# janbruedigam/ConstrainedControl.jl

Hardware: AMD Instinct MI355X
Metric: LQR sim steps/sec (whole node) on N-link cartpole batch (higher is better)
Workload: dtype f64; 1 GPU; lqr_cartpole_n_pendulum N=16 links (17 bodies), hanging-equilibrium LQR, Q=I R=1 horizon 10s, y0~U(-0.5,0.5) phi_i~U(-0.2,0.2); instances_per_gpu=8192, sim_steps=1000, record=True, parallelism=instances sharded x1, lanes_per_instance=32, lds_bytes_per_workgroup=40816, launches_per_rollout=1

## Files before the change

### constrainedcontrol.jl_amd/csrc/cclqr_chain.h

```cpp
#pragma once
#include "cclqr_dev.h"

#if defined(__HIP_DEVICE_COMPILE__)
#define SCHED_FENCE() __builtin_amdgcn_sched_barrier(0)
#else
#define SCHED_FENCE() ((void)0)
#endif
#if defined(__HIP_DEVICE_COMPILE__)
#define LDS_RD(L, i) (*(const volatile __attribute__((address_space(3))) double*)(const __attribute__((address_space(3))) double*)((L) + (i)))
#else
#define LDS_RD(L, i) ((L)[i])
#endif

namespace cclqr {

struct LinkC {
    double m, J[9], p1[3], p2[3], V12[6], qoc[4], axis[3];
    double dtm;
    double sxb, sxa;
    double fric;
    int flags;
    HD bool on() const { return (flags & 1) != 0; }
    HD bool has_a() const { return (flags & 2) != 0; }
    HD bool has_c() const { return (flags & 4) != 0; }
    HD bool rev() const { return (flags & 8) != 0; }
    HD bool valid() const { return (flags & 16) != 0; }
    HD bool live() const { return (flags & 32) != 0; }
    static const int DEAD = 64, BAD = 128;
    static const int FRIC = 256;
    HD bool has_fric() const { return (flags & FRIC) != 0; }
    static const int PRIM = 512;
    HD bool prim() const { return (flags & PRIM) != 0; }
    HD bool dead() const { return (flags & DEAD) != 0; }
    HD bool bad() const { return (flags & BAD) != 0; }
    HD void set_valid(bool v) { flags |= v ? (16 | ((flags & 1) << 5)) : 0; }
};
#if defined(__HIP_DEVICE_COMPILE__)
#define LINK_FLAGS_FRESH(c) asm volatile("" : "+v"((c).flags))
#define LANE_INT_FRESH(x) asm volatile("" : "+v"(x))
#else
#define LINK_FLAGS_FRESH(c) ((void)0)
#define LANE_INT_FRESH(x) ((void)0)
#endif

HD void link_load_consts_rec(LinkC& c, const MechDev* M, const PlantRec* P, int t, int nb, double dt) {
    const bool on = t < nb;
    const int l = on ? t : 0;
    const PlantRec* r = P + l;

    c.m = r->m;
#pragma unroll
    for (int i = 0; i < 9; i++) c.J[i] = r->J[i];
#pragma unroll
    for (int i = 0; i < 3; i++) { c.p1[i] = r->p1[i]; c.p2[i] = r->p2[i]; c.axis[i] = M->axis[l][i]; }
#pragma unroll
    for (int i = 0; i < 4; i++) c.qoc[i] = M->qoc[l][i];
    const int type = M->type[l];
    const int vrow = type == 0 ? 3 : 0;
#pragma unroll
    for (int i = 0; i < 3; i++) { c.V12[i] = M->sel[l][vrow][i]; c.V12[3 + i] = M->sel[l][vrow + 1][i]; }
    const int pa = M->parent[l];
    const bool has_a = on && pa >= 0;
    c.flags = (on ? 1 : 0) | (has_a ? 2 : 0) | ((on && M->childl[l] >= 0) ? 4 : 0) | (type == 0 ? 8 : 0);
    c.dtm = dt / c.m;
    c.sxb = dt * c.dtm;
    c.sxa = has_a ? dt * dt / P[pa >= 0 ? pa : 0].m : 0.0;
    c.fric = 0.0;
}
HD void link_load_consts(LinkC& c, const MechDev* M, int t, int nb, double dt) { link_load_consts_rec(c, M, M->rec, t, nb, dt); }
HD void row_sel(const LinkC& c, int row, double* s) {
    const bool rev = c.rev();
    const int e = rev ? row : row - 2;
    const bool unit = rev ? row < 3 : row >= 2;
    const int v = rev ? row - 3 : row;
#pragma unroll
    for (int i = 0; i < 3; i++) s[i] = unit ? (i == e ? 1.0 : 0.0) : c.V12[3 * (v & 1) + i];
}

template <bool JAC>
HD void joint_eval_sparse(const LinkC& c, const double* xa, const double* qa, const double* xb, const double* qb,
                          const double* Na, const double* Nb, double* g, double (*XT)[3], double (*PB)[3], double (*PA)[3]) {
    double Ra[9], Rb[9], rp[3], w[3], RaTw[3], gT[3];
    rotmat(qa, Ra); rotmat(qb, Rb);
    mv3(Rb, c.p2, rp);
#pragma unroll
    for (int i = 0; i < 3; i++) w[i] = xb[i] + rp[i] - xa[i];
    mtv3(Ra, w, RaTw);
#pragma unroll
    for (int i = 0; i < 3; i++) gT[i] = RaTw[i] - c.p1[i];
    double qac[4] = {qa[0], -qa[1], -qa[2], -qa[3]}, rel[4], e[4];
    qmul(qac, qb, rel);
    qmul(rel, c.qoc, e);
    const bool rot2 = !c.rev();
    if (!JAC) {
#pragma unroll
        for (int row = 0; row < 5; row++) {
            double s[3];
            row_sel(c, row, s);
            const double vT = s[0] * gT[0] + s[1] * gT[1] + s[2] * gT[2], vR = s[0] * e[1] + s[1] * e[2] + s[2] * e[3];
            g[row] = row < 2 ? vT : (row > 2 ? vR : (rot2 ? vR : vT));
        }
        return;
    }
    double RaTRb[9], PTb[9], PRb[9];
    mtm3(Ra, Rb, RaTRb);
    {
        const double* p = c.p2;
#pragma unroll
        for (int i = 0; i < 3; i++) {
            const double a = RaTRb[i * 3], b = RaTRb[i * 3 + 1], cc = RaTRb[i * 3 + 2];
            PTb[i * 3 + 0] = -2.0 * (b * p[2] - cc * p[1]);
            PTb[i * 3 + 1] = -2.0 * (cc * p[0] - a * p[2]);
            PTb[i * 3 + 2] = -2.0 * (a * p[1] - b * p[0]);
        }
    }
    {
        const double s = rel[0], x = rel[1], y = rel[2], z = rel[3];
        const double os = c.qoc[0], ox = c.qoc[1], oy = c.qoc[2], oz = c.qoc[3];
        const double Lr[3][4] = {{x, s, -z, y}, {y, z, s, -x}, {z, -y, x, s}};
        const double Rc[4][3] = {{-ox, -oy, -oz}, {os, oz, -oy}, {-oz, os, ox}, {oy, -ox, os}};
#pragma unroll
        for (int i = 0; i < 3; i++)
#pragma unroll
            for (int j = 0; j < 3; j++) PRb[i * 3 + j] = Lr[i][0] * Rc[0][j] + Lr[i][1] * Rc[1][j] + Lr[i][2] * Rc[2][j] + Lr[i][3] * Rc[3][j];
    }
// ... 167 lines not shown
    inv3(Dr, DINV);
    make_N(w2, sq2, dt, N);
    mm3(N, DINV, NB);
    return acc;
}

#define GKSZ 39
HD int gk_row(int q) { return q < 3 ? 9 * q : 27 + 6 * (q - 3); }

HD void ck_next_pose(const double* z, const double* s, double dt, double* xq) {
    const double* w2 = s + 3;
#pragma unroll
    for (int i = 0; i < 3; i++) xq[i] = z[i] + s[i] * dt;
    const double inv_dt = fast_rcp(dt);
    const double sq2 = sqrt(4.0 * inv_dt * inv_dt - (w2[0] * w2[0] + w2[1] * w2[1] + w2[2] * w2[2]));
    const double wb[4] = {0.5 * dt * sq2, 0.5 * dt * w2[0], 0.5 * dt * w2[1], 0.5 * dt * w2[2]};
    qmul(z + 3, wb, xq + 3);
}

struct SchurCol { double kx[3], kpx[3], kcx[3], kb[3], ka[3], kpb[3], kca[3]; };
HD void schur_col_load(SchurCol& K, int q, int j, int jp, int jc, const Lay& Y, const double* L) {
    const int o = gk_row(q), ob = q < 3 ? 3 : 0;
#pragma unroll
    for (int i = 0; i < 3; i++) {
        if (q < 3) { K.kx[i] = LDS_RD(L, Y.GKA + GKSZ * j + o + i); K.kpx[i] = LDS_RD(L, Y.GKA + GKSZ * jp + o + i); K.kcx[i] = LDS_RD(L, Y.GKA + GKSZ * jc + o + i); }
        else { K.kx[i] = 0.0; K.kpx[i] = 0.0; K.kcx[i] = 0.0; }
        K.kb[i] = LDS_RD(L, Y.GKA + GKSZ * j + o + ob + i); K.ka[i] = LDS_RD(L, Y.GKA + GKSZ * j + o + ob + 3 + i);
        K.kpb[i] = LDS_RD(L, Y.GKA + GKSZ * jp + o + ob + i); K.kca[i] = LDS_RD(L, Y.GKA + GKSZ * jc + o + ob + 3 + i);
    }
}
template <bool PF = false>
HD void ck_schur_rows(const LinkC& c, int j, bool store, const Lay& Y, double* L, const double (*wXT)[3], const double (*wPB)[3],
                      const double (*wPA)[3], const double* g, const double* d, const double* pd) {
    const double sx = c.sxb + c.sxa;
    const int jp = c.has_a() ? j - 1 : j, jc = c.has_c() ? j + 1 : j;
    SchurCol KA, KB;
    if (PF) schur_col_load(KA, 0, j, jp, jc, Y, L);
#pragma unroll
    for (int q = 0; q < 5; q++) {
        SchurCol& K = PF ? ((q & 1) ? KB : KA) : KA;
        if (!PF) schur_col_load(K, q, j, jp, jc, Y, L);
        else if (q < 4) { schur_col_load((q & 1) ? KA : KB, q + 1, j, jp, jc, Y, L); SCHED_FENCE(); }
        const double *kx = K.kx, *kpx = K.kpx, *kcx = K.kcx, *kb = K.kb, *ka = K.ka, *kpb = K.kpb, *kca = K.kca;
        double ojj[5], ojp[5], ojc[5];
#pragma unroll
        for (int r = 0; r < 5; r++) {
            const double bb = wPB[r][0] * kb[0] + wPB[r][1] * kb[1] + wPB[r][2] * kb[2];
            const double aa = wPA[r][0] * ka[0] + wPA[r][1] * ka[1] + wPA[r][2] * ka[2];
            const double ajp = wPA[r][0] * kpb[0] + wPA[r][1] * kpb[1] + wPA[r][2] * kpb[2];
            const double bjc = wPB[r][0] * kca[0] + wPB[r][1] * kca[1] + wPB[r][2] * kca[2];
            if (r < 3 && q < 3) {
                const double xx = wXT[r][0] * kx[0] + wXT[r][1] * kx[1] + wXT[r][2] * kx[2];
                const double xjp = wXT[r][0] * kpx[0] + wXT[r][1] * kpx[1] + wXT[r][2] * kpx[2];
                const double xjc = wXT[r][0] * kcx[0] + wXT[r][1] * kcx[1] + wXT[r][2] * kcx[2];
                ojj[r] = sx * xx + bb + aa; ojp[r] = ajp - c.sxa * xjp; ojc[r] = bjc - c.sxb * xjc;
            } else { ojj[r] = bb + aa; ojp[r] = ajp; ojc[r] = bjc; }
        }
        if (store) {
#pragma unroll
            for (int r = 0; r < 5; r++) L[Y.SJJ + 25 * j + 5 * q + r] = ojj[r];
            if (c.has_a()) {
#pragma unroll
                for (int r = 0; r < 5; r++) L[Y.SJP + 25 * j + 5 * q + r] = ojp[r];
            }
            if (c.has_c()) {
#pragma unroll
                for (int r = 0; r < 5; r++) L[Y.SPJ + 25 * jc + 5 * q + r] = ojc[r];
            }
        }
        SCHED_FENCE();
    }
    if (store) {
#pragma unroll
        for (int r = 0; r < 5; r++) {
            const double bd = wPB[r][0] * d[3] + wPB[r][1] * d[4] + wPB[r][2] * d[5];
            const double ad = wPA[r][0] * pd[3] + wPA[r][1] * pd[4] + wPA[r][2] * pd[5];
            double rr = g[r] - bd - ad;
            if (r < 3) {
                const double xd = wXT[r][0] * d[0] + wXT[r][1] * d[1] + wXT[r][2] * d[2];
                const double xa = wXT[r][0] * pd[0] + wXT[r][1] * pd[1] + wXT[r][2] * pd[2];
                rr = g[r] - (c.sxb * xd + bd) - (ad - c.sxa * xa);
            }
            L[Y.R + 5 * j + r] = rr;
        }
    }
}

template <int KL> struct SubRows { static const int NR = KL == 3 ? 2 : 3; };
struct SubSel {
    double sa[3], sb[3], s2[3];
    int w;
    int ia, ib, ic;
};
HD void row_sel_rt(const LinkC& c, int row, double* s) {
    const bool rev = c.rev();
    const bool unit = rev ? row < 3 : row >= 2;
    const int e = rev ? row : row - 2, v = rev ? row - 3 : row;
#pragma unroll
    for (int i = 0; i < 3; i++) s[i] = unit ? (i == e ? 1.0 : 0.0) : c.V12[3 * (v & 1) + i];
}
template <int KL>
HD void sub_setup(const LinkC& c, int w, SubSel& Q) {
    Q.w = w;
    const bool mid = KL == 3 && w == 2;
    row_sel_rt(c, 2, Q.s2);
    row_sel_rt(c, mid ? 2 : (w & 1), Q.sa);
    row_sel_rt(c, mid ? 2 : 3 + (w & 1), Q.sb);
    Q.ia = mid ? 2 : w;
    Q.ib = mid ? -1 : 3 + w;
    Q.ic = (KL == 2 && w == 0) ? 2 : -1;
}
template <int KL>
HD void joint_eval_rows(const LinkC& c, const SubSel& Q, const double* xa, const double* qa, const double* xb, const double* qb, const double* Na, const double* Nb,
                        double* g, double (*XT)[3], double (*PB)[3], double (*PA)[3]) {
    constexpr int NR = SubRows<KL>::NR;
    double Ra[9], Rb[9], rp[3], wv[3], RaTw[3], gT[3];
    rotmat(qa, Ra); rotmat(qb, Rb);
    mv3(Rb, c.p2, rp);
#pragma unroll
    for (int i = 0; i < 3; i++) wv[i] = xb[i] + rp[i] - xa[i];
    mtv3(Ra, wv, RaTw);
#pragma unroll
    for (int i = 0; i < 3; i++) gT[i] = RaTw[i] - c.p1[i];
    double qac[4] = {qa[0], -qa[1], -qa[2], -qa[3]}, rel[4], e[4];
    qmul(qac, qb, rel);
    qmul(rel, c.qoc, e);
    double RaTRb[9], PTb[9], PRb[9];
    mtm3(Ra, Rb, RaTRb);
    {
        const double* p = c.p2;
#pragma unroll
        for (int i = 0; i < 3; i++) {
            const double a = RaTRb[i * 3], b = RaTRb[i * 3 + 1], cc = RaTRb[i * 3 + 2];
            PTb[i * 3 + 0] = -2.0 * (b * p[2] - cc * p[1]);
            PTb[i * 3 + 1] = -2.0 * (cc * p[0] - a * p[2]);
            PTb[i * 3 + 2] = -2.0 * (a * p[1] - b * p[0]);
        }
    }
    {
        const double s = rel[0], x = rel[1], y = rel[2], z = rel[3];
        const double os = c.qoc[0], ox = c.qoc[1], oy = c.qoc[2], oz = c.qoc[3];
        const double Lr[3][4] = {{x, s, -z, y}, {y, z, s, -x}, {z, -y, x, s}};
        const double Rc[4][3] = {{-ox, -oy, -oz}, {os, oz, -oy}, {-oz, os, ox}, {oy, -ox, os}};
#pragma unroll
        for (int i = 0; i < 3; i++)
#pragma unroll
            for (int j = 0; j < 3; j++) PRb[i * 3 + j] = Lr[i][0] * Rc[0][j] + Lr[i][1] * Rc[1][j] + Lr[i][2] * Rc[2][j] + Lr[i][3] * Rc[3][j];
    }
    const double PTa[9] = {0, -2 * RaTw[2], 2 * RaTw[1], 2 * RaTw[2], 0, -2 * RaTw[0], -2 * RaTw[1], 2 * RaTw[0], 0};
    const double PRa[9] = {-e[0], -e[3], e[2], e[3], -e[0], -e[1], -e[2], e[1], -e[0]};
    const bool rot2 = !c.rev();
    double pb3[NR][3], pa3[NR][3];
    {
        const double a0 = Q.sa[0], a1 = Q.sa[1], a2 = Q.sa[2], b0 = Q.sb[0], b1 = Q.sb[1], b2 = Q.sb[2];
        const double vT = a0 * gT[0] + a1 * gT[1] + a2 * gT[2], vR = b0 * e[1] + b1 * e[2] + b2 * e[3];
        int wq = Q.w;
        LANE_INT_FRESH(wq);
        const bool merge = KL == 3 && wq == 2;
        const bool rot = merge && rot2;
        g[0] = rot ? vR : vT;
        g[1] = merge ? 0.0 : vR;
#pragma unroll
        for (int k = 0; k < 3; k++) {
            const double xt = a0 * Ra[k * 3] + a1 * Ra[k * 3 + 1] + a2 * Ra[k * 3 + 2];
            const double ptb = a0 * PTb[k] + a1 * PTb[3 + k] + a2 * PTb[6 + k], pta = a0 * PTa[k] + a1 * PTa[3 + k] + a2 * PTa[6 + k];
            const double prb = b0 * PRb[k] + b1 * PRb[3 + k] + b2 * PRb[6 + k], pra = b0 * PRa[k] + b1 * PRa[3 + k] + b2 * PRa[6 + k];
// ... 438 lines not shown
```

### constrainedcontrol.jl_amd/csrc/rollout_chain.hip

```cpp
#include "cclqr_chain.h"
#include "cclqr_internal.h"
#include "cclqr_newton.h"
#include "cclqr_rollout_step.h"

namespace cclqr {

__device__ __forceinline__ double wave_from_prev(double v) {
    int lo = __double2loint(v), hi = __double2hiint(v);
    lo = __builtin_amdgcn_update_dpp(0, lo, 0x138, 0xf, 0xf, true);
    hi = __builtin_amdgcn_update_dpp(0, hi, 0x138, 0xf, 0xf, true);
    return __hiloint2double(hi, lo);
}
__device__ __forceinline__ double wave_from_next(double v) {
    int lo = __double2loint(v), hi = __double2hiint(v);
    lo = __builtin_amdgcn_update_dpp(0, lo, 0x130, 0xf, 0xf, true);
    hi = __builtin_amdgcn_update_dpp(0, hi, 0x130, 0xf, 0xf, true);
    return __hiloint2double(hi, lo);
}
template <int N>
__device__ __forceinline__ void from_prev(const double* in, double* out) {
#pragma unroll
    for (int i = 0; i < N; i++) out[i] = wave_from_prev(in[i]);
}
template <int N>
__device__ __forceinline__ void from_next(const double* in, double* out) {
#pragma unroll
    for (int i = 0; i < N; i++) out[i] = wave_from_next(in[i]);
}

__device__ __forceinline__ void ck_tri_mid_regs(int t, bool done, const TriPlanB& B, const TriCur& K, const Lay& Y, const double* L, const double* tg, double* dl, TriBack0& Q) {
    const TriPlan& P = B.P;
    ck_tri_back0_load(Q, t, done, B, K, Y, L);
    double m[5];
    const bool ran = K.n == P.steps;
#pragma unroll
    for (int r = 0; r < 5; r++) m[r] = ran ? tg[r] : 0.0;
    if (P.steps == 0) {
        asm volatile("");
        const bool f0 = (t & 8) == 0;
#pragma unroll
        for (int r = 0; r < 5; r++) m[r] = f0 ? Q.z[r] : 0.0;
    }
#pragma unroll
    for (int r = 0; r < 5; r++) m[r] = m[r] + dpp_row_ror<8>(m[r]);
    double A[25];
#pragma unroll
    for (int i = 0; i < 5; i++) {
        A[i * 5 + 0] = dpp_f64<0x150>(m[i]); A[i * 5 + 1] = dpp_f64<0x151>(m[i]); A[i * 5 + 2] = dpp_f64<0x152>(m[i]);
        A[i * 5 + 3] = dpp_f64<0x153>(m[i]); A[i * 5 + 4] = dpp_f64<0x154>(m[i]);
        dl[i] = dpp_f64<0x155>(m[i]);
    }
    lu5_factor(A);
    lu5_solve(A, dl);
}

template <int G, bool JAC, int KL = 1>
__device__ __forceinline__ double chain_eval(LinkC& c, LinkS& S, int t, const Lay& Y, double* L, double alpha, bool active, bool rows, double dt, const SubSel& Q PROF_ARG) {
    double part = 0.0;
    double NB[9], g[5], xq[7];
    const bool store_dinv = JAC && __any(rows);
    LINK_FLAGS_FRESH(c);
#pragma unroll
    for (int k = 0; k < 7; k++) xq[k] = S.z[k];
    if (active) {
        double cf[6], sv[6], cTR[6], DINV[9];
#pragma unroll
        for (int k = 0; k < 6; k++) { cf[k] = L[Y.C + 6 * t + k] - alpha * S.cd[k]; sv[k] = S.s[k] - alpha * S.ds[k]; cTR[k] = L[Y.D + 6 * t + k]; }
        part = ck_body_eval<JAC>(c, S.z, sv, cf, cTR, cTR + 3, dt, xq, S.d, DINV, NB);
        if (KL > 1 && !c.prim()) part = 0.0;
        if (store_dinv && (KL == 1 || c.prim())) {
#pragma unroll
            for (int k = 0; k < 9; k++) L[Y.DINV + 9 * t + k] = DINV[k];
        }
    }
    STAMP(PF_EVAL_BODY);
    double pxq[7], pNB[9];
    from_prev<7>(xq, pxq);
    if (JAC) from_prev<9>(NB, pNB);
    if (!c.has_a()) {
#pragma unroll
        for (int i = 0; i < 7; i++) pxq[i] = (i == 3) ? 1.0 : 0.0;
    }
    if (JAC && KL > 1) {
        constexpr int NR = SubRows<KL>::NR;
        double gs[NR], sXT[NR][3], sPB[NR][3], sPA[NR][3];
        if (active) {
            joint_eval_rows<KL>(c, Q, pxq, pxq + 3, xq, xq + 3, pNB, NB, gs, sXT, sPB, sPA);
#pragma unroll
            for (int i = 0; i < NR; i++) part += gs[i] * gs[i];
        }
        STAMP(PF_EVAL_JOINT);
        LINK_FLAGS_FRESH(c);
        if (__any(rows)) {
            double pd[6];
            from_prev<6>(S.d, pd);
            ck_schur_rows_sub<KL, (KL == 3)>(c, Q, t, active, Y, L, gs, sXT, sPB, sPA, S.d, pd);
        } else {
            PCOUNT(PF_ROWS_SKIPPED);
        }
        STAMP(PF_SCHUR_S);
    } else {
        double wXT[3][3], wPB[5][3], wPA[5][3];
        if (active) {
            joint_eval_sparse<JAC>(c, pxq, pxq + 3, xq, xq + 3, pNB, NB, g, wXT, wPB, wPA);
            if (KL == 1) {
#pragma unroll
                for (int i = 0; i < 5; i++) part += g[i] * g[i];
            } else {
                double pj = 0.0;
#pragma unroll
                for (int i = 0; i < 5; i++) pj += g[i] * g[i];
                part += c.prim() ? pj : 0.0;
            }
        }
        STAMP(PF_EVAL_JOINT);
        LINK_FLAGS_FRESH(c);
        if (JAC) {
            if (__any(rows)) {
                double pd[6];
                from_prev<6>(S.d, pd);
                ck_schur_rows(c, t, active, Y, L, wXT, wPB, wPA, g, S.d, pd);
            } else {
                PCOUNT(PF_ROWS_SKIPPED);
            }
            STAMP(PF_SCHUR_S);
        }
    }
    const double nrm = sqrt(group_sum<G>(part));
    STAMP(PF_EVAL_MAP);
    PCOUNT(PF_EVALS);
    return nrm;
}

template <int G, int KL = 1>
__device__ __forceinline__ void chain_eval2(LinkC& c, const TrialIn& T, const double* Lc, int t, const Lay& Y, double a1, double a2, bool active, double dt,
                                            double& n1, double& n2) {
    double part1 = 0.0, part2 = 0.0, xq1[7], xq2[7];
    LINK_FLAGS_FRESH(c);
#pragma unroll
    for (int k = 0; k < 7; k++) { xq1[k] = T.z[k]; xq2[k] = T.z[k]; }
    if (active) {
        double cf1[6], cf2[6], sv1[6], sv2[6], cTR[6], d1[6], d2[6];
#pragma unroll
        for (int k = 0; k < 6; k++) {
            const double cc = Lc[Y.C + 6 * t + k];
            cTR[k] = Lc[Y.D + 6 * t + k];
            cf1[k] = cc - a1 * T.cd[k]; cf2[k] = cc - a2 * T.cd[k];
            sv1[k] = T.s[k] - a1 * T.ds[k]; sv2[k] = T.s[k] - a2 * T.ds[k];
        }
        part1 = ck_body_eval<false>(c, T.z, sv1, cf1, cTR, cTR + 3, dt, xq1, d1, nullptr, nullptr);
        part2 = ck_body_eval<false>(c, T.z, sv2, cf2, cTR, cTR + 3, dt, xq2, d2, nullptr, nullptr);
    }
    double p1[7], p2[7];
    from_prev<7>(xq1, p1);
    from_prev<7>(xq2, p2);
    if (!c.has_a()) {
#pragma unroll
        for (int i = 0; i < 7; i++) { p1[i] = (i == 3) ? 1.0 : 0.0; p2[i] = p1[i]; }
    }
    if (active) {
        double g1[5], g2[5];
        joint_eval_sparse<false>(c, p1, p1 + 3, xq1, xq1 + 3, nullptr, nullptr, g1, (double(*)[3]) nullptr, (double(*)[3]) nullptr, (double(*)[3]) nullptr);
        joint_eval_sparse<false>(c, p2, p2 + 3, xq2, xq2 + 3, nullptr, nullptr, g2, (double(*)[3]) nullptr, (double(*)[3]) nullptr, (double(*)[3]) nullptr);
#pragma unroll
        for (int i = 0; i < 5; i++) { part1 += g1[i] * g1[i]; part2 += g2[i] * g2[i]; }
    }
    if (KL > 1 && !c.prim()) { part1 = 0.0; part2 = 0.0; }
    n1 = sqrt(group_sum<G>(part1));
    n2 = sqrt(group_sum<G>(part2));
}

template <int G, int KL = 1>
__device__ __forceinline__ double chain_eval1(LinkC& c, const TrialIn& T, const double* Lc, int t, const Lay& Y, double a1, bool active, double dt) {
    double part1 = 0.0, xq1[7];
    LINK_FLAGS_FRESH(c);
#pragma unroll
    for (int k = 0; k < 7; k++) xq1[k] = T.z[k];
    if (active) {
        double cf1[6], sv1[6], cTR[6], d1[6];
#pragma unroll
        for (int k = 0; k < 6; k++) {
            cTR[k] = Lc[Y.D + 6 * t + k];
            cf1[k] = Lc[Y.C + 6 * t + k] - a1 * T.cd[k];
            sv1[k] = T.s[k] - a1 * T.ds[k];
        }
        part1 = ck_body_eval<false>(c, T.z, sv1, cf1, cTR, cTR + 3, dt, xq1, d1, nullptr, nullptr);
    }
    double p1[7];
    from_prev<7>(xq1, p1);
    if (!c.has_a()) {
#pragma unroll
        for (int i = 0; i < 7; i++) p1[i] = (i == 3) ? 1.0 : 0.0;
    }
    if (active) {
        double g1[5];
        joint_eval_sparse<false>(c, p1, p1 + 3, xq1, xq1 + 3, nullptr, nullptr, g1, (double(*)[3]) nullptr, (double(*)[3]) nullptr, (double(*)[3]) nullptr);
#pragma unroll
        for (int i = 0; i < 5; i++) part1 += g1[i] * g1[i];
    }
    if (KL > 1 && !c.prim()) part1 = 0.0;
    return sqrt(group_sum<G>(part1));
}
__device__ __forceinline__ double lane_fetch(double v, int addr) {
    return __hiloint2double(__builtin_amdgcn_ds_bpermute(addr, __double2hiint(v)), __builtin_amdgcn_ds_bpermute(addr, __double2loint(v)));
}

__device__ __attribute__((noinline)) double philox_normal_dev(unsigned key0, unsigned long long instance, int k) { return philox_normal(key0, instance, k); }
__global__ __launch_bounds__(256) void philox_fill_kernel(double* out, unsigned key0, long long inst0, long long n_inst, int k0, int steps) {
    const long long i = (long long)blockIdx.x * 256 + threadIdx.x;
    if (i >= n_inst * steps) return;
    const long long n = i / steps;
    const int kk = (int)(i - n * steps);
    out[i] = philox_normal_dev(key0, (unsigned long long)(inst0 + n), k0 + kk);
}
hipError_t launch_philox_fill(double* out, unsigned key0, long long inst0, long long n_inst, int k0, int steps, hipStream_t stream) {
    const long long total = n_inst * steps;
    if (total <= 0) return hipSuccess;
    return launch_lds<false>(philox_fill_kernel, dim3((unsigned)((total + 255) / 256)), dim3(256), 0, stream, out, key0, inst0, n_inst, k0, steps);
}

template <int G, int NBP, int EXTRA, bool RELAX = false, int KL = 1, int NL = G>
__global__ __launch_bounds__(WAVE_BLOCK) void rollout_chain_kernel(RolloutArgs a) {
    extern __shared__ double lds[];
    static_assert(WAVE_BLOCK == 64, "WAVE_HANDOVER orders the phases of ONE wavefront: the workgroup is exactly 64 threads");
    static_assert(KL >= 1 && KL <= 3 && KL * NL <= G && (KL > 1 || NL == G) && (KL == 1 || NL <= NBP), "lane group too small for KL lanes per link");
    const int lane = threadIdx.x, t = lane % G, grp = lane / G;
    const int w = KL > 1 ? t / NL : 0;
    const int tl = KL > 1 ? t - NL * w : t;
    const int tc = KL > 1 ? (w < KL ? tl : -2) : t;
    const int64_t inst = (int64_t)blockIdx.x * a.ipw + grp;
    const MechDev* M = a.M;
    const CtrlDev* CT = a.C;
    const int nb = M->nb;
    const double dt = M->dt;
    const Lay Y = make_chain_layout(NBP);
    double* L = lds + grp * Y.total;
    const int nz = 13 * nb;

    LinkC c;
    const PlantRec* plant = M->rec;
    const bool have = grp < a.ipw && inst < a.n_inst;
    if (a.plants) plant = a.plants + ((unsigned)a.plant_off + (have ? (unsigned)inst : 0u)) * (unsigned)nb;
    link_load_consts_rec(c, M, plant, (KL > 1 && w >= KL) ? CCLQR_MAXL : tl, nb, dt);
    if (KL == 1 || w == 0) c.flags |= LinkC::PRIM;
    SubSel Q;
    if (KL > 1) sub_setup<KL>(c, w < KL ? w : 0, Q);
    if (EXTRA && CT->has_fric && c.on()) { c.fric = CT->fric[tl]; if (c.fric != 0.0) c.flags |= LinkC::FRIC; }
    c.set_valid(have);
    const long long ginst = a.inst0 + inst;
    const int ut = c.on() ? M->perm[tl] : 0;
    int plan;
    {
        const int nch = M->nchains;
        const int cs = M->chain_start[lane], cn = M->chain_len[lane];
        plan = chain_plan_pack(nch, lane < nch ? cs : 0, lane < nch ? cn : 0) | (ut << 24);
    }

    LinkS S;
    double pid_int = 0.0, pid_last = 0.0;
#pragma unroll
    for (int i = 0; i < 7; i++) S.z[i] = c.live() ? a.z0[inst * nz + ut * 13 + i] : ((i == 3) ? 1.0 : 0.0);
#pragma unroll
    for (int i = 0; i < 6; i++) S.s[i] = c.live() ? a.z0[inst * nz + ut * 13 + 7 + i] : 0.0;
    if (EXTRA == 2 && a.pid_state && a.k0 > 1 && c.live()) { pid_int = a.pid_state[(inst * nb + tl) * 2]; pid_last = a.pid_state[(inst * nb + tl) * 2 + 1]; }
#pragma unroll
    for (int i = 0; i < 6; i++) { S.cd[i] = 0.0; S.d[i] = 0.0; S.ds[i] = 0.0; }
    if (c.on() && (KL == 1 || c.prim())) {
        const bool warm = c.live() && a.lam && a.k0 > 1;
#pragma unroll
        for (int i = 0; i < 5; i++) L[Y.LAM + 5 * tl + i] = warm ? a.lam[inst * 5 * nb + 5 * tl + i] : 0.0;
    }
    WAVE_HANDOVER();

#ifdef CCLQR_PROFILE
    Prof prof;
    prof.start();
#endif
    int worst = 0;
    if (a.carry && a.status && c.valid()) {
        const NewtonStatus st = status_decode(a.status[inst]);
        worst = st.worst;
        if (st.bad) c.flags |= LinkC::BAD;
        if (st.dead) c.flags |= LinkC::DEAD;
    }
    typedef const __attribute__((address_space(4))) RolloutArgs* KernArgs;
    KernArgs ap = (KernArgs)__builtin_amdgcn_kernarg_segment_ptr();
    const int k0 = a.k0;
    int nsteps = a.steps;
    for (int kk = 0; kk < nsteps; kk++) {
        const int k = k0 + kk;
        asm volatile("" : "+s"(ap));
        LINK_FLAGS_FRESH(c);
        CtrlHotK C = ctrl_hot_of(CT);
        asm volatile("" : "+s"(C));
        const long long gi = c.valid() ? ginst : a.inst0;
        const int ne = 12 * nb;
        const int mu = C->mu;
        const CtrlRows rows = ctrl_step_rows(C, k, gi, nz, ne);
        const bool gate = rows.gate;
        const GlobalD Kp = global_table(C->K) + rows.K + t;
        const GlobalD Fp = C->Fd ? global_table(C->Fd) + rows.Fd : (GlobalD)0;
        double grav = M->g;
        unsigned long long zd_base = C->zd;
        asm volatile("" : "+s"(zd_base));
        double* const traj_out = ap->traj;
        if (traj_out) {
            if (c.live() && (KL == 1 || c.prim())) {
                LANE_INT_FRESH(plan);
                const int ub = plan >> 24;
#pragma unroll
                for (int i = 0; i < 7; i++) L[Y.Z + 13 * ub + i] = S.z[i];
#pragma unroll
                for (int i = 0; i < 6; i++) L[Y.Z + 13 * ub + 7 + i] = S.s[i];
            }
        }
        STAMP(PF_IO);
        double uj = 0.0;
        double zf[13], za[13];
#pragma unroll
        for (int i = 0; i < 7; i++) zf[i] = S.z[i];
#pragma unroll
        for (int i = 0; i < 6; i++) zf[7 + i] = S.s[i];
        from_prev<7>(zf, za);
        if (EXTRA) from_prev<6>(zf + 7, za + 7);
        if (!c.has_a()) {
#pragma unroll
            for (int i = 0; i < 13; i++) za[i] = (i == 3) ? 1.0 : 0.0;
// ... 9 lines not shown
#pragma unroll
                    for (int i = 0; i < 12; i++) L[Y.DZ + 12 * tl + i] = dz[i];
                }
                if (EXTRA && (C->flags & CtrlHot::FRIC) && c.has_fric()) uj = ck_friction(c, zf, za);
            }
        }
        WAVE_HANDOVER();
        if (gate) {
            constexpr int NE = GainRows<G, NBP>::NE;
            double unoise = 0.0;
            if (EXTRA == 3) {
                if (C->flags & CtrlHot::NOISE) unoise = C->noise_scale * philox_normal_dev(C->noise_key0, (unsigned long long)gi, k);
            } else if (EXTRA) {
                const double* noise = ap->noise;
                if ((C->flags & CtrlHot::NOISE) && c.valid() && noise) unoise = C->noise_scale * noise[(size_t)inst * ap->noise_stride + (k - 1)];
            }
            double dzv[NE];
            int tf = t;
            asm volatile("" : "+v"(tf));
#pragma unroll
            for (int q = 0; q < NE; q++) { const int e = tf + q * G; dzv[q] = (c.valid() && e < ne) ? L[Y.DZ + e] : 0.0; }
            feedback_inputs<G, NBP, EXTRA>(C, Kp, Fp, mu, ne, dzv, unoise, tc, uj);
        }
        STAMP(PF_CONTROL);
        asm volatile("" : "+v"(grav));
        if (traj_out) {
            if (c.valid()) {
                int kr = kk, nzr = nz;
                asm volatile("" : "+s"(kr), "+s"(nzr));
                double* dst = traj_out + ((size_t)inst * ap->steps + kr) * nzr;
                int e0 = t;
                asm volatile("" : "+v"(e0));
                for (int e = e0; e < nz; e += G) dst[e] = L[Y.Z + e];
            }
        }
        STAMP(PF_IO);
        if (EXTRA == 2 && (C->flags & CtrlHot::PID)) {
            if (c.live() && CT->pid_on[tl]) uj += ck_pid(c, zf, za, CT->pid_P[tl], CT->pid_I[tl], CT->pid_D[tl], CT->pid_goal[tl], dt, k == 1, pid_int, pid_last);
        }
        STAMP(PF_CONTROL);
        LINK_FLAGS_FRESH(c);
        {
            double F[3], tau[3], W6[6], cW6[6];
            ck_joint_wrench(c, uj, zf + 3, za + 3, F, tau, W6, W6 + 3);
            from_next<6>(W6, cW6);
            if (c.has_c()) {
#pragma unroll
                for (int i = 0; i < 3; i++) { F[i] += cW6[i]; tau[i] += cW6[3 + i]; }
            }
            double cTR[6];
            ck_step_invariants(c, zf, F, tau, dt, grav, cTR, cTR + 3);
            double gk[5], kXT[3][3], kPB[5][3], kPA[5][3], lam[5];
            joint_eval_sparse<true>(c, za, za + 3, zf, zf + 3, nullptr, nullptr, gk, kXT, kPB, kPA);
#pragma unroll
            for (int i = 0; i < 5; i++) lam[i] = L[Y.LAM + 5 * tl + i];
            if (c.live() && (KL == 1 || c.prim())) {
                gk_store(tl, Y, L, kXT, kPB, kPA);
#pragma unroll
                for (int i = 0; i < 6; i++) L[Y.D + 6 * tl + i] = cTR[i];
            }
            double own[6], par[6], cpar[6];
            jac_t_apply(c, kXT, kPB, kPA, lam, own, par);
            from_next<6>(par, cpar);
#pragma unroll
            for (int i = 0; i < 6; i++) S.cd[i] = 0.0;
            if (c.live() && (KL == 1 || c.prim())) {
#pragma unroll
                for (int i = 0; i < 6; i++) L[Y.C + 6 * tl + i] = own[i] + (c.has_c() ? cpar[i] : 0.0);
            }
        }
        WAVE_HANDOVER();

        STAMP(PF_FORCES);
        PCOUNT(PF_STEPS);
        const bool go = c.valid() && !c.dead();
        bool done = !go, failed = false;
        int its = 0;
        double normf0 = 0.0;
        LANE_INT_FRESH(plan);
        const int nchains = chain_plan_count(__builtin_amdgcn_readfirstlane(plan));
        bool need_jac = !done;
        for (int iter = 1; iter <= NEWTON_MAXIT; iter++) {
            if (__any(need_jac)) {
                const double nf = chain_eval<G, true, KL>(c, S, tl, Y, L, 0.0, c.live() && need_jac, need_jac, dt, Q PROF_PASS);
                if (iter == 1) normf0 = nf;
            }
            WAVE_HANDOVER();
            if (!__any(!done)) break;
            PCOUNT(PF_NEWTON_ITERS);
            const bool active = c.live() && !done;
            for (int ci = 0; ci < nchains; ci++) {
                const int pw = __builtin_amdgcn_readlane(plan, ci);
                const int cs = chain_plan_start(pw), cn = chain_plan_len(pw);
                constexpr int CRW = 4;
                constexpr bool CR = G == 32 && NBP <= 17;
                const bool cr = CR && cn >= CR_MIN_LINKS;
                if (CR && cr) {
                    CrLane<CRW> CK;
                    double tc[CrLane<CRW>::NS][5];
                    cr_setup<CRW>(CK, t, cs, cn, 1, Y, done);
                    CR_FLAGS_FRESH(CK);
                    cr_phase_a<CRW>(CK, L, tc);
                    CR_FLAGS_FRESH(CK);
                    cr_store_a<CRW>(CK, L, tc);
                    WAVE_HANDOVER();
                    CR_FLAGS_FRESH(CK);
                    cr_phase_b<CRW>(CK, L, tc);
                    CR_FLAGS_FRESH(CK);
                    cr_store_b<CRW>(CK, L, tc);
                    WAVE_HANDOVER();
                }
                STAMP(PF_SCHUR_W);
                const TriPlanB PB = cr ? tri_plan_balanced(cs, (cn + 1) / 2, 2) : tri_plan_balanced(cs, cn, 1, G >= 16 ? 2 : 1);
                const TriPlan& P = PB.P;
                TriCur K = tri_cursor(t, PB, Y);
                if (done) K.n = 0;
                if constexpr (G >= 16) {
                    double tg[5] = {0.0, 0.0, 0.0, 0.0, 0.0}, dlm[5];
                    for (int i = 0; i < P.steps; i++) {
                        double zy[5];
                        int otg = 0, oout = 0;
                        int left = P.steps - 1 - i;
                        LANE_INT_FRESH(left);
                        if (tri_step(K, i, L, tg, zy, &otg, &oout)) tri_step_store_fold(L, otg, oout, tg, zy, left == 0);
                        WAVE_HANDOVER();
                    }
                    STAMP(PF_TRI_FWD);
                    TriBack0 B0;
                    ck_tri_mid_regs(t, done, PB, K, Y, L, tg, dlm, B0);
                    ck_tri_back0_store(B0, t, Y, L, dlm);
                    WAVE_HANDOVER();
                    for (int j = 1; j < P.steps; j++) {
                        if (!done) ck_tri_back(t, j, PB, Y, L);
                        WAVE_HANDOVER();
                    }
                    if (!done && t == 0) {
#pragma unroll
                        for (int i = 0; i < 5; i++) L[Y.DL + 5 * P.mid + i] = dlm[i];
                    }
                    WAVE_HANDOVER();
                } else {
                    for (int i = 0; i < P.steps; i++) {
                        double tg[5], zy[5];
                        int otg = 0, oout = 0;
                        if (tri_step(K, i, L, tg, zy, &otg, &oout)) tri_step_store(L, otg, oout, tg, zy);
                        WAVE_HANDOVER();
                    }
                    STAMP(PF_TRI_FWD);
                    if (!done) ck_tri_mid<false>(t, PB, Y, L);
                    WAVE_HANDOVER();
                    for (int j = 0; j < P.steps; j++) {
                        if (!done) ck_tri_back(t, j, PB, Y, L);
                        WAVE_HANDOVER();
                    }
                }
                if (CR && cr) {
                    cr_back<CRW>(t, cs, cn, 1, Y, L, done);
                    WAVE_HANDOVER();
                }
                STAMP(PF_TRI_BWD);
            }
            double nd;
            LINK_FLAGS_FRESH(c);
            {
                double own[6], par[6], cpar[6], dl[5], pdn = 0.0;
#pragma unroll
                for (int r = 0; r < 5; r++) dl[r] = L[Y.DL + 5 * tl + r];
                gk_t_apply<true>(c, tl, Y, L, dl, own, par);
                from_next<6>(par, cpar);
                if (active) {
                    double DINV[9];
#pragma unroll
                    for (int i = 0; i < 9; i++) DINV[i] = L[Y.DINV + 9 * tl + i];
#pragma unroll
                    for (int i = 0; i < 6; i++) S.cd[i] = own[i] + (c.has_c() ? cpar[i] : 0.0);
                    ck_body_solve(c, S.d, S.cd, DINV, S.ds);
#pragma unroll
                    for (int i = 0; i < 6; i++) pdn += S.ds[i] * S.ds[i];
#pragma unroll
                    for (int i = 0; i < 5; i++) pdn += dl[i] * dl[i];
                    if (KL > 1 && !c.prim()) pdn = 0.0;
                }
                nd = sqrt(group_sum<G>(pdn));
            }
            WAVE_HANDOVER();
            STAMP(PF_BODY_SOLVE);
            double alpha = 1.0, normf1 = 0.0;
            const bool want_rows = !done && !(normf0 < NEWTON_EPS && nd < NEWTON_EPS);
            bool ls_done = done, jac_ok = __any(want_rows);
            {
                const double nf = chain_eval<G, true, KL>(c, S, tl, Y, L, 1.0, active, want_rows, dt, Q PROF_PASS);
                if (!ls_done) {
                    normf1 = nf;
                    if (!(normf1 > normf0)) ls_done = true;
                }
            }
            if (G == 32) {
                for (int lv = 1; lv <= LINE_MAXIT;) {
                    if (!__any(!ls_done)) break;
                    const bool mine = !ls_done;
                    const bool other = __shfl_xor(mine ? 1 : 0, 32, 64) != 0;
                    const bool solo = ap->plants != nullptr;
                    const bool helping = !mine && other && !solo;
                    TrialIn T;
#pragma unroll
                    for (int i = 0; i < 7; i++) T.z[i] = S.z[i];
#pragma unroll
                    for (int i = 0; i < 6; i++) { T.s[i] = S.s[i]; T.ds[i] = S.ds[i]; T.cd[i] = S.cd[i]; }
                    if (mine != other) {
#pragma unroll
                        for (int i = 0; i < 7; i++) { const double o = other_half(S.z[i]); T.z[i] = helping ? o : T.z[i]; }
#pragma unroll
                        for (int i = 0; i < 6; i++) {
                            const double o1 = other_half(S.s[i]), o2 = other_half(S.ds[i]), o3 = other_half(S.cd[i]);
                            T.s[i] = helping ? o1 : T.s[i]; T.ds[i] = helping ? o2 : T.ds[i]; T.cd[i] = helping ? o3 : T.cd[i];
                        }
                    }
                    const double* Lc = helping ? lds + (1 - grp) * Y.total : L;
                    const int l0 = helping ? lv + 2 : lv;
                    double n1, n2;
                    chain_eval2<G, KL>(c, T, Lc, tl, Y, ldexp(1.0, -l0), ldexp(1.0, -(l0 + 1)), c.on() && (mine || helping) && l0 <= LINE_MAXIT, dt, n1, n2);
                    PCOUNT(PF_EVALS);
                    const double h1 = other_half(n1), h2 = other_half(n2);
                    if (mine) {
                        const double cand[4] = {n1, n2, h1, h2};
#pragma unroll
                        for (int i = 0; i < 4; i++) {
                            const int l = lv + i;
                            if (!ls_done && l <= LINE_MAXIT && (i < 2 || !(other || solo))) {
                                normf1 = cand[i]; alpha = ldexp(1.0, -l); jac_ok = false;
                                if (!(cand[i] > normf0) || l == LINE_MAXIT) ls_done = true;
                            }
                        }
                    }
                    lv += (solo || (mine && other)) ? 2 : 4;
                }
            } else {
                constexpr int NG = 64 / G;
                for (int lv = 1; lv <= LINE_MAXIT;) {
                    if (!__any(!ls_done)) break;
                    const bool mine = !ls_done;
                    const unsigned long long heads = __ballot(mine && t == 0);
                    const bool solo = ap->plants != nullptr;
                    const int count = solo ? NG : __builtin_popcountll(heads);
                    const int per = NG / count;
                    const int kq = grp % count, off = grp / count;
                    unsigned long long hm = heads;
                    for (int i = 0; i < kq; i++) hm &= hm - 1;
                    const int src = solo ? grp : __builtin_ctzll(hm) / G;
                    int myrank = 0;
                    for (int g2 = 0; g2 < NG; g2++) myrank += (g2 < grp && ((heads >> (g2 * G)) & 1ull)) ? 1 : 0;
                    const int l0 = lv + off;
                    const bool work = off < per && l0 <= LINE_MAXIT;
                    const int fa = (src * G + t) * 4;
                    TrialIn T;
#pragma unroll
                    for (int i = 0; i < 7; i++) T.z[i] = S.z[i];
#pragma unroll
                    for (int i = 0; i < 6; i++) { T.s[i] = S.s[i]; T.ds[i] = S.ds[i]; T.cd[i] = S.cd[i]; }
                    if (count < NG) {
#pragma unroll
                        for (int i = 0; i < 7; i++) T.z[i] = lane_fetch(S.z[i], fa);
#pragma unroll
                        for (int i = 0; i < 6; i++) { T.s[i] = lane_fetch(S.s[i], fa); T.ds[i] = lane_fetch(S.ds[i], fa); T.cd[i] = lane_fetch(S.cd[i], fa); }
                    }
                    const double nf = chain_eval1<G, KL>(c, T, lds + src * Y.total, tl, Y, ldexp(1.0, -l0), c.on() && work, dt);
                    PCOUNT(PF_EVALS);
                    if (count == NG) {
                        if (mine) {
                            normf1 = nf; alpha = ldexp(1.0, -lv); jac_ok = false;
                            if (!(nf > normf0) || lv == LINE_MAXIT) ls_done = true;
                        }
                    } else {
#pragma unroll
// ... 137 lines not shown
```

Baseline: 28.95 million instance-steps/s.

## Split Schur row assembly across idle lanes in 32-lane chain groups

For 17-body chains on 32-lane groups, idle upper lanes become helpers that take half of each link's Schur-complement block work. Joint Jacobian weights are swapped across 16-lane rows with permlane16_swap, and a new split routine writes the diagonal and off-diagonal blocks from separate lanes. The aim is to shorten the per-lane critical path of the row assembly. In exchange it adds cross-lane swaps, a root special case and more complex indexing, which risks register pressure and correctness issues.

```diff
diff --git a/constrainedcontrol.jl_amd/csrc/cclqr_chain.h b/constrainedcontrol.jl_amd/csrc/cclqr_chain.h
--- a/constrainedcontrol.jl_amd/csrc/cclqr_chain.h
+++ b/constrainedcontrol.jl_amd/csrc/cclqr_chain.h
@@ -31,6 +31,9 @@
     HD bool has_fric() const { return (flags & FRIC) != 0; }
     static const int PRIM = 512;
     HD bool prim() const { return (flags & PRIM) != 0; }
+    static const int HELP = 1024, HELPC = 2048;
+    HD bool help() const { return (flags & HELP) != 0; }
+    HD bool help_c() const { return (flags & HELPC) != 0; }
     HD bool dead() const { return (flags & DEAD) != 0; }
     HD bool bad() const { return (flags & BAD) != 0; }
     HD void set_valid(bool v) { flags |= v ? (16 | ((flags & 1) << 5)) : 0; }
@@ -38,9 +41,11 @@
 #if defined(__HIP_DEVICE_COMPILE__)
 #define LINK_FLAGS_FRESH(c) asm volatile("" : "+v"((c).flags))
 #define LANE_INT_FRESH(x) asm volatile("" : "+v"(x))
+#define LANE_F64_FRESH(x) asm volatile("" : "+v"(x))
 #else
 #define LINK_FLAGS_FRESH(c) ((void)0)
 #define LANE_INT_FRESH(x) ((void)0)
+#define LANE_F64_FRESH(x) ((void)0)
 #endif
 
 HD void link_load_consts_rec(LinkC& c, const MechDev* M, const PlantRec* P, int t, int nb, double dt) {
@@ -374,6 +379,81 @@
                 rr = g[r] - (c.sxb * xd + bd) - (ad - c.sxa * xa);
             }
             L[Y.R + 5 * j + r] = rr;
+        }
+    }
+}
+
+HD void schur_split_helper(LinkC& c, bool has_child, double sxb_link) {
+    c.flags |= LinkC::HELP | (has_child ? LinkC::HELPC : 0);
+    c.sxb = -sxb_link; c.sxa = -0.0;
+}
+template <bool R0>
+HD void ck_schur_rows_split(const LinkC& c, int t, bool store, bool gstore, const Lay& Y, double* L, const double (*wXT)[3], const double (*wPB)[3],
+                            double (*wPA)[3], const double* g, const double* d, const double* pd) {
+    const bool help = c.help(), root = R0 && t == 0, plain = !help && !root;
+    const int jc = t - (help ? 16 : 0) + ((c.flags >> (help ? 11 : 2)) & 1);
+    const int j1 = help ? jc : t, j3 = plain ? t - ((c.flags >> 1) & 1) : jc;
+    const int x1 = Y.GKA + GKSZ * j1, p1 = x1 + (help ? 3 : 0);
+    const int x3 = Y.GKA + GKSZ * j3, p3 = x3 + (root ? 3 : 0);
+    const int o1 = (help ? Y.SPJ : Y.SJJ) + 25 * j1, o3 = (root ? Y.SPJ + 25 * jc : Y.SJP + 25 * t);
+    const bool st1 = help ? (gstore && c.help_c()) : store, st3 = root ? c.has_c() : c.has_a();
+    const double s1 = c.sxb + c.sxa, s3 = root ? -c.sxb : -c.sxa;
+    double z0 = help ? -0.0 : 0.0;
+    LANE_F64_FRESH(z0);
+    if (R0 && root) {
+#pragma unroll
+        for (int r = 0; r < 5; r++)
+#pragma unroll
+            for (int k = 0; k < 3; k++) wPA[r][k] = wPB[r][k];
+    }
+    const double (*wP3)[3] = wPA;
+#pragma unroll
+    for (int q = 0; q < 5; q++) {
+        const int o = gk_row(q), ob = q < 3 ? 3 : 0;
+        double kx1[3], kx3[3], k1[3], ka[3], k3[3];
+#pragma unroll
+        for (int i = 0; i < 3; i++) {
+            if (q < 3) { kx1[i] = LDS_RD(L, x1 + o + i); kx3[i] = LDS_RD(L, x3 + o + i); }
+            else { kx1[i] = 0.0; kx3[i] = 0.0; }
+            k1[i] = LDS_RD(L, p1 + o + ob + i); ka[i] = LDS_RD(L, x1 + o + ob + 3 + i); k3[i] = LDS_RD(L, p3 + o + ob + i);
+        }
+        double u1[5], u3[5];
+#pragma unroll
+        for (int r = 0; r < 5; r++) {
+            const double bb = wPB[r][0] * k1[0] + wPB[r][1] * k1[1] + wPB[r][2] * k1[2];
+            const double aa = wP3[r][0] * ka[0] + wP3[r][1] * ka[1] + wP3[r][2] * ka[2];
+            const double ajp = wP3[r][0] * k3[0] + wP3[r][1] * k3[1] + wP3[r][2] * k3[2];
+            const double z = plain ? aa : z0;
+            if (r < 3 && q < 3) {
+                const double xx = wXT[r][0] * kx1[0] + wXT[r][1] * kx1[1] + wXT[r][2] * kx1[2];
+                const double xjp = wXT[r][0] * kx3[0] + wXT[r][1] * kx3[1] + wXT[r][2] * kx3[2];
+                const double u = s1 * xx + bb;
+                u1[r] = u + z; u3[r] = ajp + s3 * xjp;
+            } else { u1[r] = bb + z; u3[r] = ajp; }
+        }
+        if (st1) {
+#pragma unroll
+            for (int r = 0; r < 5; r++) L[o1 + 5 * q + r] = u1[r];
+            if (st3) {
+#pragma unroll
+                for (int r = 0; r < 5; r++) L[o3 + 5 * q + r] = u3[r];
+            }
+        }
+        SCHED_FENCE();
+    }
+    if (store) {
+#pragma unroll
+        for (int r = 0; r < 5; r++) {
+            const double bd = wPB[r][0] * d[3] + wPB[r][1] * d[4] + wPB[r][2] * d[5];
+            double ad = wP3[r][0] * pd[3] + wP3[r][1] * pd[4] + wP3[r][2] * pd[5];
+            if (R0) ad = root ? 0.0 : ad;
+            double rr = g[r] - bd - ad;
+            if (r < 3) {
+                const double xd = wXT[r][0] * d[0] + wXT[r][1] * d[1] + wXT[r][2] * d[2];
+                const double xa = wXT[r][0] * pd[0] + wXT[r][1] * pd[1] + wXT[r][2] * pd[2];
+                rr = g[r] - (c.sxb * xd + bd) - (ad - c.sxa * xa);
+            }
+            L[Y.R + 5 * t + r] = rr;
         }
     }
 }
diff --git a/constrainedcontrol.jl_amd/csrc/rollout_chain.hip b/constrainedcontrol.jl_amd/csrc/rollout_chain.hip
--- a/constrainedcontrol.jl_amd/csrc/rollout_chain.hip
+++ b/constrainedcontrol.jl_amd/csrc/rollout_chain.hip
@@ -54,8 +54,40 @@
     lu5_solve(A, dl);
 }
 
-template <int G, bool JAC, int KL = 1>
-__device__ __forceinline__ double chain_eval(LinkC& c, LinkS& S, int t, const Lay& Y, double* L, double alpha, bool active, bool rows, double dt, const SubSel& Q PROF_ARG) {
+__device__ __forceinline__ auto swap_rows_b32(unsigned first, unsigned second) { return __builtin_amdgcn_permlane16_swap(first, second, false, false); }
+template <bool KEEP, int N>
+__device__ __forceinline__ void from_row_below(double* v, bool keep) {
+    double cp[N];
+#pragma unroll
+    for (int i = 0; i < N; i++) { cp[i] = v[i]; asm volatile("" : "+v"(cp[i])); }
+#pragma unroll
+    for (int i = 0; i < N; i++) {
+        const auto a = swap_rows_b32((unsigned)__double2loint(cp[i]), (unsigned)__double2loint(v[i]));
+        const auto b = swap_rows_b32((unsigned)__double2hiint(cp[i]), (unsigned)__double2hiint(v[i]));
+        const unsigned lo = KEEP ? (keep ? a[1] : a[0]) : a[0], hi = KEEP ? (keep ? b[1] : b[0]) : b[0];
+        v[i] = __hiloint2double((int)hi, (int)lo);
+    }
+}
+template <int G, int NBP, int KL> struct SchurSplit { static const bool ON = G == 32 && NBP <= 17 && KL == 1, R0 = NBP == 17; };
+template <int NBP>
+__device__ __forceinline__ void schur_split_setup(LinkC& c, int t, const MechDev* M, int nb) {
+    const int l = t & 15;
+    const bool help = t >= 16 && !c.on();
+    double sl = c.sxb;
+    from_row_below<false, 1>(&sl, false);
+    if (help) schur_split_helper(c, l < nb && M->childl[l] >= 0, sl);
+}
+template <bool R0>
+__device__ __forceinline__ void schur_split_take(const LinkC& c, int t, double (*wXT)[3], double (*wPB)[3]) {
+    const bool keep = R0 && t >= 16 && !c.help();
+#pragma unroll
+    for (int r = 0; r < 3; r++) from_row_below<R0, 3>(wXT[r], keep);
+#pragma unroll
+    for (int r = 0; r < 5; r++) from_row_below<R0, 3>(wPB[r], keep);
+}
+
+template <int G, bool JAC, int KL = 1, int SP = 0>
+__device__ __forceinline__ double chain_eval(LinkC& c, LinkS& S, int t, const Lay& Y, double* L, double alpha, bool active, bool inst_on, bool rows, double dt, const SubSel& Q PROF_ARG) {
     double part = 0.0;
     double NB[9], g[5], xq[7];
     const bool store_dinv = JAC && __any(rows);
@@ -101,6 +133,16 @@
         STAMP(PF_SCHUR_S);
     } else {
         double wXT[3][3], wPB[5][3], wPA[5][3];
+        if constexpr (JAC && SP != 0) {
+#pragma unroll
+            for (int r = 0; r < 3; r++)
+#pragma unroll
+                for (int k = 0; k < 3; k++) asm volatile("" : "=v"(wXT[r][k]));
+#pragma unroll
+            for (int r = 0; r < 5; r++)
+#pragma unroll
+                for (int k = 0; k < 3; k++) asm volatile("" : "=v"(wPB[r][k]));
+        }
         if (active) {
             joint_eval_sparse<JAC>(c, pxq, pxq + 3, xq, xq + 3, pNB, NB, g, wXT, wPB, wPA);
             if (KL == 1) {
@@ -119,7 +161,12 @@
             if (__any(rows)) {
                 double pd[6];
                 from_prev<6>(S.d, pd);
-                ck_schur_rows(c, t, active, Y, L, wXT, wPB, wPA, g, S.d, pd);
+                if constexpr (SP != 0) {
+                    schur_split_take<SP == 2>(c, t, wXT, wPB);
+                    ck_schur_rows_split<SP == 2>(c, t, active, inst_on, Y, L, wXT, wPB, wPA, g, S.d, pd);
+                } else {
+                    ck_schur_rows(c, t, active, Y, L, wXT, wPB, wPA, g, S.d, pd);
+                }
             } else {
                 PCOUNT(PF_ROWS_SKIPPED);
             }
@@ -243,6 +290,8 @@
     if (a.plants) plant = a.plants + ((unsigned)a.plant_off + (have ? (unsigned)inst : 0u)) * (unsigned)nb;
     link_load_consts_rec(c, M, plant, (KL > 1 && w >= KL) ? CCLQR_MAXL : tl, nb, dt);
     if (KL == 1 || w == 0) c.flags |= LinkC::PRIM;
+    constexpr int SP = SchurSplit<G, NBP, KL>::ON ? (SchurSplit<G, NBP, KL>::R0 ? 2 : 1) : 0;
+    if constexpr (SP != 0) schur_split_setup<NBP>(c, t, M, nb);
     SubSel Q;
     if (KL > 1) sub_setup<KL>(c, w < KL ? w : 0, Q);
     if (EXTRA && CT->has_fric && c.on()) { c.fric = CT->fric[tl]; if (c.fric != 0.0) c.flags |= LinkC::FRIC; }
@@ -418,7 +467,7 @@
         bool need_jac = !done;
         for (int iter = 1; iter <= NEWTON_MAXIT; iter++) {
             if (__any(need_jac)) {
-                const double nf = chain_eval<G, true, KL>(c, S, tl, Y, L, 0.0, c.live() && need_jac, need_jac, dt, Q PROF_PASS);
+                const double nf = chain_eval<G, true, KL, SP>(c, S, tl, Y, L, 0.0, c.live() && need_jac, need_jac, need_jac, dt, Q PROF_PASS);
                 if (iter == 1) normf0 = nf;
             }
             WAVE_HANDOVER();
@@ -525,7 +574,7 @@
             const bool want_rows = !done && !(normf0 < NEWTON_EPS && nd < NEWTON_EPS);
             bool ls_done = done, jac_ok = __any(want_rows);
             {
-                const double nf = chain_eval<G, true, KL>(c, S, tl, Y, L, 1.0, active, want_rows, dt, Q PROF_PASS);
+                const double nf = chain_eval<G, true, KL, SP>(c, S, tl, Y, L, 1.0, active, !done, want_rows, dt, Q PROF_PASS);
                 if (!ls_done) {
                     normf1 = nf;
                     if (!(normf1 > normf0)) ls_done = true;
```

New measurement: 29.58 million instance-steps/s, median of 6. 1.02x the previous value.
